# likojack/bnv_fusion

Hardware: AMD Instinct MI355X
Metric: depth frames/sec fused+decoded, 640x480 @ 256^3 grid (higher is better)
Workload: dtype f32 operands split into f16 hi+lo, 3 products on v_mfma_f32_16x16x32_f16, f32 accumulate

## Files before the change

### bnv_fusion_amd/csrc/encode.hip

```cpp
#include <stddef.h>

#include <atomic>
#include <utility>
#include <vector>

#include "frontend.hpp"
#include "tcnn_mlp.hpp"

namespace bnv {

int g_num_cus = 0;
int g_last_hip_error = 0;
std::atomic<int> g_reserve_cus{0};
std::atomic<int> g_finalize_blocks{0};
std::atomic<int> g_tcnn_shared_table{1};
std::atomic<int> g_tcnn_block_encoder{1};
std::atomic<int> g_mlp_mode{1};

bool g_prof_on = false;
static std::vector<std::pair<hipEvent_t, hipEvent_t>> g_prof_events[PROF_KINDS];
static size_t g_prof_used[PROF_KINDS] = {0, 0, 0, 0};

void prof_mark(int kind, bool begin, hipStream_t stream) {
  auto& ring = g_prof_events[kind];
// ... 827 lines not shown
    const bool have = tile_pair(T, t, j, &i, &k);
    float in0 = 0.f, in1 = 0.f, in2 = 0.f;
    int slot = -1;
    bool valid = false;
    if (have) {
      const float* p = pts + (size_t)i * 6;
      const float x = p[0], y = p[1], z = p[2];
      valid = in_bounds(x, y, z, g);
      if (valid) {
        const float xn = voxel_coord(x, g.bound_min[0], g.voxel_size);
        const float yn = voxel_coord(y, g.bound_min[1], g.voxel_size);
        const float zn = voxel_coord(z, g.bound_min[2], g.voxel_size);
        const int gx = (k & 1) ? (int)ceilf(xn) : (int)floorf(xn);
        const int gy = (k & 2) ? (int)ceilf(yn) : (int)floorf(yn);
        const int gz = (k & 4) ? (int)ceilf(zn) : (int)floorf(zn);
        if (voxel_owner(gx, gy, gz, g) == g.shard_rank) {
          const uint32_t id = (uint32_t)(gx * nyz + gy * g.n_xyz[2] + gz);
          const uint32_t word = bitmap[id >> 5];
          slot = (int)(word_prefix[id >> 5] + __popc(word & ((1u << (id & 31)) - 1u)));
        }
        const float rx = relative_coord(xn, gx, g.voxel_size);
        const float ry = relative_coord(yn, gy, g.voxel_size);
        const float rz = relative_coord(zn, gz, g.voxel_size);
        in0 = h ? ry : rx;
        in1 = h ? p[3] : rz;
        in2 = h ? p[5] : p[4];
      }
    }
    if (__ballot(slot >= 0) == 0ULL) continue;

    f32x16 ha[4], hb[4];
#pragma unroll
    for (int mb = 0; mb < 4; ++mb) ha[mb] = bias_init(lds + PN_B1, mb, h);
    {
      const float bin[3] = {in0, in1, in2};
#pragma unroll
      for (int s = 0; s < 3; ++s) {
#pragma unroll
        for (int mb = 0; mb < 4; ++mb)
          ha[mb] = __builtin_amdgcn_mfma_f32_32x32x2f32(lds[PN_W1 + (s * 4 + mb) * 64 + lane], bin[s],
                                                        ha[mb], 0, 0, 0);
      }
    }
#pragma unroll
    for (int mb = 0; mb < 4; ++mb) ha[mb] = relu16(ha[mb]);
    layer128(lds + PN_W2, lds + PN_B2, ha, hb, lane, h);
#pragma unroll
    for (int mb = 0; mb < 4; ++mb) hb[mb] = relu16(hb[mb]);
    layer128(lds + PN_W3, lds + PN_B3, hb, ha, lane, h);
#pragma unroll
    for (int mb = 0; mb < 4; ++mb) ha[mb] = relu16(ha[mb]);
    f32x16 o;
#pragma unroll
    for (int r = 0; r < 16; ++r) o[r] = 0.f;
    {
      const f32x4 b4 = *(const f32x4*)&lds[PN_B4 + 4 * h];
#pragma unroll
      for (int r = 0; r < 4; ++r) o[r] = b4[r];
    }
#pragma unroll
    for (int nb = 0; nb < 4; ++nb) {
#pragma unroll
      for (int rq = 0; rq < 4; ++rq) {
        f32x4 a = {0.f, 0.f, 0.f, 0.f};
        if (j < 8) a = *(const f32x4*)&lds[PN_W4 + ((((nb * 4 + rq) * 2 + h) * 8) + j) * 4];
#pragma unroll
        for (int i = 0; i < 4; ++i)
          o = __builtin_amdgcn_mfma_f32_32x32x2f32(a[i], ha[nb][4 * rq + i], o, 0, 0, 0);
      }
    }
    scatter_tile(o, slot, j, h, counts, acc);
  }
}


typedef __attribute__((address_space(3))) const half8 lds_half8_t;
typedef __attribute__((address_space(3))) const f32x4 lds_f32x4_t;
constexpr int kLdsWin = 61440;

#ifdef BNV_PHASE_PROF
__device__ unsigned long long g_enc_phase[8 * 16];
#define BNV_EPH(i)                                                                          \
  do {                                                                                      \
    if ((threadIdx.x & 63) == 0) {                                                          \
      unsigned long long* _p = (unsigned long long*)((char*)lds + PX_LDS_BYTES) + (threadIdx.x >> 6) * 16; \
      const unsigned long long _t = clock64();                                              \
      _p[i] += _t - _p[15];                                                                 \
      _p[15] = _t;                                                                          \
    }                                                                                       \
  } while (0)
constexpr int kEncProfLds = 8 * 16 * 8;
#else
#define BNV_EPH(i)
constexpr int kEncProfLds = 0;
#endif

struct EncLdsX {
  uint32_t w[3];
  uint32_t b;
};
__device__ __forceinline__ half8 ldsx_wfrag(const EncLdsX& L, int byte_off) {
  const int b = byte_off / kLdsWin;
  return *(lds_half8_t*)((b == 0 ? L.w[0] : (b == 1 ? L.w[1] : L.w[2])) + (uint32_t)(byte_off - b * kLdsWin));
}
__device__ __forceinline__ f32x4 ldsx_bias(const EncLdsX& L, int layer, int rb) {
  return *(lds_f32x4_t*)(L.b + (uint32_t)((layer * 128 + rb * 16) * 4));
}

template <int NPROD>
__device__ __forceinline__ void layer128_x(const EncLdsX& L, int w_off, int layer, const half8 (&inh)[4][2],
                                           const half8 (&inl)[4][2], f32x4 (&out)[8][2]) {
#pragma unroll
  for (int rb = 0; rb < 8; ++rb) out[rb][0] = out[rb][1] = ldsx_bias(L, layer, rb);
  half8 ah[2], al[2];
#define BNV_LOAD_WX(q)                                                        \
  {                                                                           \
    const int wb = (w_off + (q) * 2 * 64 * 8) * 2;                            \
    ah[(q) & 1] = ldsx_wfrag(L, wb);                                          \
    if (NPROD == 3) al[(q) & 1] = ldsx_wfrag(L, wb + 1024);                   \
  }
  BNV_LOAD_WX(0);
#pragma unroll
  for (int q = 0; q < 32; ++q) {
    if (q + 1 < 32) BNV_LOAD_WX(q + 1);
    __builtin_amdgcn_sched_barrier(0);
    const int s = q >> 3, rb = q & 7;
    if constexpr (NPROD == 3) {
      out[rb][0] = __builtin_amdgcn_mfma_f32_16x16x32_f16(al[q & 1], inh[s][0], out[rb][0], 0, 0, 0);
      out[rb][1] = __builtin_amdgcn_mfma_f32_16x16x32_f16(al[q & 1], inh[s][1], out[rb][1], 0, 0, 0);
      out[rb][0] = __builtin_amdgcn_mfma_f32_16x16x32_f16(ah[q & 1], inl[s][0], out[rb][0], 0, 0, 0);
      out[rb][1] = __builtin_amdgcn_mfma_f32_16x16x32_f16(ah[q & 1], inl[s][1], out[rb][1], 0, 0, 0);
    }
    out[rb][0] = __builtin_amdgcn_mfma_f32_16x16x32_f16(ah[q & 1], inh[s][0], out[rb][0], 0, 0, 0);
    out[rb][1] = __builtin_amdgcn_mfma_f32_16x16x32_f16(ah[q & 1], inh[s][1], out[rb][1], 0, 0, 0);
    __builtin_amdgcn_sched_barrier(0);
  }
#undef BNV_LOAD_WX
}

template <int NPROD>
__device__ __forceinline__ void split_x(const f32x4 (&acc)[8][2], half8 (&oh)[4][2], half8 (&ol)[4][2]) {
#pragma unroll
  for (int s = 0; s < 4; ++s)
#pragma unroll
    for (int cb = 0; cb < 2; ++cb) {
      float x[8];
#pragma unroll
      for (int e = 0; e < 8; ++e) x[e] = relu_bits(acc[2 * s + (e >> 2)][cb][e & 3]);
      if (NPROD == 3) {
        split8_f16(x, oh[s][cb], ol[s][cb]);
      } else {
#pragma unroll
        for (int e = 0; e < 8; ++e) oh[s][cb][e] = (_Float16)x[e];
      }
    }
}

__device__ __forceinline__ void scatter_tile_x(const f32x4& o, int slot, int n, int g, int32_t* __restrict__ counts,
                                               long long* __restrict__ acc) {
  uint32_t lo[4], hi[4];
#pragma unroll
  for (int q = 0; q < 4; ++q) {
    const float r = __builtin_rintf(o[q] * kFixedScale);
    const float hf = __builtin_floorf(r * (1.0f / kFixedScale));
    hi[q] = (uint32_t)(int)hf;
    lo[q] = (uint32_t)__builtin_fmaf(hf, -kFixedScale, r);
  }
#define BNV_SCAN_STEP(ctrl)                                                      \
  "v_add_co_u32_dpp %0, vcc, %0, %0 " ctrl "\n"                                  \
  "v_addc_co_u32_dpp %1, vcc, %1, %1, vcc " ctrl "\n"                            \
  "v_add_co_u32_dpp %2, vcc, %2, %2 " ctrl "\n"                                  \
  "v_addc_co_u32_dpp %3, vcc, %3, %3, vcc " ctrl "\n"                            \
  "v_add_co_u32_dpp %4, vcc, %4, %4 " ctrl "\n"                                  \
  "v_addc_co_u32_dpp %5, vcc, %5, %5, vcc " ctrl "\n"                            \
  "v_add_co_u32_dpp %6, vcc, %6, %6 " ctrl "\n"                                  \
  "v_addc_co_u32_dpp %7, vcc, %7, %7, vcc " ctrl "\n"
  asm volatile("s_nop 1\n"
               BNV_SCAN_STEP("row_shr:1 row_mask:0xf bank_mask:0xf bound_ctrl:1")
               BNV_SCAN_STEP("row_shr:2 row_mask:0xf bank_mask:0xf bound_ctrl:1")
               BNV_SCAN_STEP("row_shr:4 row_mask:0xf bank_mask:0xf bound_ctrl:1")
               BNV_SCAN_STEP("row_shr:8 row_mask:0xf bank_mask:0xf bound_ctrl:1")
               : "+v"(lo[0]), "+v"(hi[0]), "+v"(lo[1]), "+v"(hi[1]), "+v"(lo[2]), "+v"(hi[2]), "+v"(lo[3]), "+v"(hi[3])
               :
               : "vcc");
#undef BNV_SCAN_STEP
  {
    const int tsrc = ((g & 1) * 16 + 15) * 4;
#pragma unroll
    for (int q = 0; q < 4; ++q) {
      const uint32_t tl = (uint32_t)__builtin_amdgcn_ds_bpermute(tsrc, (int)lo[q]);
      const uint32_t th = (uint32_t)__builtin_amdgcn_ds_bpermute(tsrc, (int)hi[q]);
      if (g >= 2) {
        const unsigned long long v = (((unsigned long long)hi[q] << 32) | lo[q]) + (((unsigned long long)th << 32) | tl);
        lo[q] = (uint32_t)v;
        hi[q] = (uint32_t)(v >> 32);
      }
    }
  }
  const int p = (g >> 1) * 16 + n;
  const int slot15 = __builtin_amdgcn_readlane(slot, 15);
  const int prev_row = __builtin_amdgcn_update_dpp(0, slot, 0x111 , 0xf, 0xf, false);
  const int prev = n == 0 ? slot15 : prev_row;
  const unsigned long long heads64 = __ballot(p == 0 || prev != slot);
  const uint32_t heads = ((uint32_t)heads64 & 0xffffu) | (((uint32_t)(heads64 >> 32) & 0xffffu) << 16);
  const int s = 31 - __clz((int)(heads & (0xffffffffu >> (31 - p))));
  const bool is_end = p == 31 || ((heads >> (p + 1)) & 1u);
  const int sp = s > 0 ? s - 1 : 0;
  const int src = (((sp >> 4) * 2 + (g & 1)) * 16 + (sp & 15)) * 4;
  uint32_t plo[4], phi[4];
#pragma unroll
  for (int q = 0; q < 4; ++q) {
    plo[q] = (uint32_t)__builtin_amdgcn_ds_bpermute(src, (int)lo[q]);
    phi[q] = (uint32_t)__builtin_amdgcn_ds_bpermute(src, (int)hi[q]);
  }
#ifdef BNV_PROBE_NO_SCATTER
  if ((blockIdx.x & 63) != 0) return;
#endif
  if (slot >= 0 && is_end) {
    unsigned long long* dst = (unsigned long long*)acc + ((uint32_t)slot * 8u + 4u * (uint32_t)(g & 1));
#pragma unroll
    for (int q = 0; q < 4; ++q) {
      unsigned long long v = ((unsigned long long)hi[q] << 32) | lo[q];
      if (s > 0) v -= ((unsigned long long)phi[q] << 32) | plo[q];
      atomicAdd(dst + q, v);
    }
    if ((g & 1) == 0) atomicAdd(&counts[slot], p - s + 1);
  }
}

template <int NPROD>
__global__ __launch_bounds__(512, 2) __attribute__((amdgpu_num_vgpr(120))) void k_pointnet_scatter_x(
    const float* __restrict__ pts, int n_points, bnv_grid_t g, const float* __restrict__ wpack,
    const uint32_t* __restrict__ bitmap, const uint32_t* __restrict__ word_prefix,
    int32_t* __restrict__ counts, long long* __restrict__ acc, int32_t* __restrict__ error,
    const int32_t* __restrict__ pair_list, const int32_t* __restrict__ n_pairs) {
  extern __shared__ __attribute__((aligned(16))) float lds[];
  const float n_cert = wpack[PN_CERT];
  float* lb = lds + PX_TOTAL / 2;
  for (int i = threadIdx.x; i < 128 * 3 + 8; i += 512) lb[i] = wpack[PN_B1 + i];
  stage_to_lds<512>(wpack + PX_OFF, lds, PX_TOTAL * 2);
  int* tile_ctr = (int*)((char*)lds + PX_TOTAL * 2 + (128 * 3 + 8) * 4);
  if (threadIdx.x == 0) *tile_ctr = 0;
  __syncthreads();

  const int lane = threadIdx.x & 63;
  const int n = lane & 15, gk = lane >> 4;
  const int pair = (gk >> 1) * 16 + n;
  const PairTiles T = pair_tiles(n_points, pair_list, n_pairs);
  const int n_tiles = T.n_tiles;
  const int nyz = g.n_xyz[1] * g.n_xyz[2];
  EncLdsX L;
  {
    const uint32_t lds0 = (uint32_t)(uintptr_t)(__attribute__((address_space(3))) float*)lds;
    L.w[0] = lds0 + lane * 16;
    L.w[1] = L.w[0] + kLdsWin;
    L.w[2] = L.w[0] + 2 * kLdsWin;
    L.b = lds0 + PX_TOTAL * 2 + gk * 16;
    asm volatile("" : "+v"(L.w[0]), "+v"(L.w[1]), "+v"(L.w[2]), "+v"(L.b));
  }

  const int tstep = gridDim.x * 8;
  auto grab = [&]() -> int {
    int c = 0;
    if (lane == 0) c = atomicAdd(tile_ctr, 1);
    c = __builtin_amdgcn_readfirstlane(c);
    return blockIdx.x * 8 + (c & 7) + (c >> 3) * tstep;
  };
  float raw[6];
  int raw_k = 0;
  bool raw_ok = false;
  float nin[6];
  uint32_t n_id = 0, n_word = 0, n_pref = 0;
  bool n_own = false;
  auto stage1 = [&](int t) {
    raw_ok = false;
    if (t < n_tiles) {
      int i = 0;
      if (tile_pair(T, t, pair, &i, &raw_k)) {
        const float* p = pts + (size_t)i * 6;
#pragma unroll
        for (int c = 0; c < 6; ++c) raw[c] = p[c];
        raw_ok = true;
      }
    }
  };
  auto stage2 = [&](int t) {
    n_own = false;
#pragma unroll
    for (int c = 0; c < 6; ++c) nin[c] = 0.f;
    if (raw_ok && in_bounds(raw[0], raw[1], raw[2], g)) {
      const int k = raw_k;
      const float xn = voxel_coord(raw[0], g.bound_min[0], g.voxel_size);
      const float yn = voxel_coord(raw[1], g.bound_min[1], g.voxel_size);
      const float zn = voxel_coord(raw[2], g.bound_min[2], g.voxel_size);
      const int gx = (k & 1) ? (int)ceilf(xn) : (int)floorf(xn);
      const int gy = (k & 2) ? (int)ceilf(yn) : (int)floorf(yn);
      const int gz = (k & 4) ? (int)ceilf(zn) : (int)floorf(zn);
      if (voxel_owner(gx, gy, gz, g) == g.shard_rank) {
        n_own = true;
        n_id = (uint32_t)(gx * nyz + gy * g.n_xyz[2] + gz);
        n_word = bitmap[n_id >> 5];
        n_pref = word_prefix[n_id >> 5];
      }
      if ((gk & 1) == 0) {
        nin[0] = relative_coord(xn, gx, g.voxel_size);
        nin[1] = relative_coord(yn, gy, g.voxel_size);
        nin[2] = relative_coord(zn, gz, g.voxel_size);
        nin[3] = raw[3];
        nin[4] = raw[4];
        nin[5] = raw[5];
      }
      if (!(fmaxf(fmaxf(fabsf(raw[3]), fabsf(raw[4])), fabsf(raw[5])) <= n_cert)) *error = 3;
    }
  };
  int t = grab();
  stage1(t);
  stage2(t);
  int t_next = grab(), t_next2 = 0;
  stage1(t_next);
#ifdef BNV_PHASE_PROF
  if ((threadIdx.x & 63) < 16)
    ((unsigned long long*)((char*)lds + PX_LDS_BYTES))[(threadIdx.x >> 6) * 16 + (threadIdx.x & 63)] = 0;
  if ((threadIdx.x & 63) == 0) ((unsigned long long*)((char*)lds + PX_LDS_BYTES))[(threadIdx.x >> 6) * 16 + 15] = clock64();
#endif

  for (; t < n_tiles; t = t_next, t_next = t_next2) {
    float in[6];
#pragma unroll
    for (int c = 0; c < 6; ++c) in[c] = nin[c];
    const int slot = n_own ? (int)(n_pref + __popc(n_word & ((1u << (n_id & 31)) - 1u))) : -1;
    stage2(t_next);
    t_next2 = grab();
    stage1(t_next2);
    __builtin_amdgcn_sched_barrier(0);
    BNV_EPH(0);
    if (__ballot(slot >= 0) == 0ULL) continue;

    f32x4 ha[8][2], hb[8][2];
    {
      half8 bh[2], bl[2];
#pragma unroll
      for (int cb = 0; cb < 2; ++cb) {
        float x[8];
#pragma unroll
        for (int e = 0; e < 8; ++e) x[e] = 0.f;
#pragma unroll
        for (int e = 0; e < 6; ++e) {
          const float other = __shfl(in[e], (lane + 32) & 63, 64);
          x[e] = gk == 0 ? (cb == 0 ? in[e] : other) : 0.f;
        }
        if (NPROD == 3) {
          split8_f16(x, bh[cb], bl[cb]);
        } else {
#pragma unroll
          for (int e = 0; e < 8; ++e) bh[cb][e] = (_Float16)x[e];
        }
      }
#pragma unroll
      for (int rb = 0; rb < 8; ++rb) {
        const half8 ahi = ldsx_wfrag(L, (PX_W1 + rb * 2 * 64 * 8) * 2), alo = ldsx_wfrag(L, (PX_W1 + rb * 2 * 64 * 8) * 2 + 1024);
        const f32x4 b = ldsx_bias(L, 0, rb);
#pragma unroll
        for (int cb = 0; cb < 2; ++cb) {
          f32x4 c = b;
          if constexpr (NPROD == 3) {
            c = __builtin_amdgcn_mfma_f32_16x16x32_f16(alo, bh[cb], c, 0, 0, 0);
            c = __builtin_amdgcn_mfma_f32_16x16x32_f16(ahi, bl[cb], c, 0, 0, 0);
          }
          ha[rb][cb] = __builtin_amdgcn_mfma_f32_16x16x32_f16(ahi, bh[cb], c, 0, 0, 0);
        }
      }
    }
    BNV_EPH(1);
    half8 sh[4][2], sl[4][2];
    split_x<NPROD>(ha, sh, sl);
    BNV_EPH(2);
    layer128_x<NPROD>(L, PX_W2, 1, sh, sl, hb);
    BNV_EPH(3);
    split_x<NPROD>(hb, sh, sl);
    BNV_EPH(4);
    layer128_x<NPROD>(L, PX_W3, 2, sh, sl, ha);
    BNV_EPH(5);
    split_x<NPROD>(ha, sh, sl);
    BNV_EPH(6);
    f32x4 o[2];
    o[0] = o[1] = *(lds_f32x4_t*)(L.b + 384 * 4);
    {
      half8 w4h[4], w4l[4];
      __builtin_amdgcn_sched_barrier(0);
#pragma unroll
      for (int s = 0; s < 4; ++s) {
        w4h[s] = ldsx_wfrag(L, (PX_W4 + s * 2 * 64 * 8) * 2);
        if (NPROD == 3) w4l[s] = ldsx_wfrag(L, (PX_W4 + s * 2 * 64 * 8) * 2 + 1024);
      }
#pragma unroll
      for (int s = 0; s < 4; ++s) {
#pragma unroll
        for (int cb = 0; cb < 2; ++cb) {
          if constexpr (NPROD == 3) {
            o[cb] = __builtin_amdgcn_mfma_f32_16x16x32_f16(w4l[s], sh[s][cb], o[cb], 0, 0, 0);
            o[cb] = __builtin_amdgcn_mfma_f32_16x16x32_f16(w4h[s], sl[s][cb], o[cb], 0, 0, 0);
          }
          o[cb] = __builtin_amdgcn_mfma_f32_16x16x32_f16(w4h[s], sh[s][cb], o[cb], 0, 0, 0);
        }
      }
    }
    f32x4 mine;
#pragma unroll
    for (int i = 0; i < 4; ++i) {
      const float other = __shfl(o[1][i], (lane + 32) & 63, 64);
      mine[i] = gk < 2 ? o[0][i] : other;
    }
    BNV_EPH(7);
    scatter_tile_x(mine, slot, n, gk, counts, acc);
    BNV_EPH(8);
  }
#ifdef BNV_PHASE_PROF
  if ((threadIdx.x & 63) < 15)
    atomicAdd(&g_enc_phase[(threadIdx.x >> 6) * 16 + (threadIdx.x & 63)],
              ((unsigned long long*)((char*)lds + PX_LDS_BYTES))[(threadIdx.x >> 6) * 16 + (threadIdx.x & 63)]);
#endif
}

typedef TcnnPack<1> PointPack;

__global__ __launch_bounds__(256) void k_pointnet_scatter_t(
    const float* __restrict__ pts, int n_points, bnv_grid_t g, const float* __restrict__ wpack,
    const uint32_t* __restrict__ bitmap, const uint32_t* __restrict__ word_prefix,
    int32_t* __restrict__ counts, long long* __restrict__ acc, const int32_t* __restrict__ pair_list,
    const int32_t* __restrict__ n_pairs) {
  __shared__ __attribute__((aligned(16))) _Float16 wh[PointPack::TOTAL];
  stage_to_lds<256>(wpack, wh, PointPack::TOTAL * 2);
  __syncthreads();
  const int lane = threadIdx.x & 63;
  const int wave = __builtin_amdgcn_readfirstlane(threadIdx.x >> 6);
  const int j = lane & 31, h = lane >> 5;
  const PairTiles T = pair_tiles(n_points, pair_list, n_pairs);
  const int n_tiles = T.n_tiles;
  const int nyz = g.n_xyz[1] * g.n_xyz[2];
  for (int t = blockIdx.x * 4 + wave; t < n_tiles; t += gridDim.x * 4) {
    int i = 0, k = 0;
    const bool have = tile_pair(T, t, j, &i, &k);
    half8 b;
#pragma unroll
    for (int e = 0; e < 8; ++e) b[e] = (_Float16)1.0f;
    int slot = -1;
    bool valid = false;
    if (have) {
      const float* p = pts + (size_t)i * 6;
      const float x = p[0], y = p[1], z = p[2];
      if (in_bounds(x, y, z, g)) {
        valid = true;
        const float xn = voxel_coord(x, g.bound_min[0], g.voxel_size);
        const float yn = voxel_coord(y, g.bound_min[1], g.voxel_size);
        const float zn = voxel_coord(z, g.bound_min[2], g.voxel_size);
        const int gx = (k & 1) ? (int)ceilf(xn) : (int)floorf(xn);
        const int gy = (k & 2) ? (int)ceilf(yn) : (int)floorf(yn);
        const int gz = (k & 4) ? (int)ceilf(zn) : (int)floorf(zn);
        if (voxel_owner(gx, gy, gz, g) == g.shard_rank) {
          const uint32_t id = (uint32_t)(gx * nyz + gy * g.n_xyz[2] + gz);
          const uint32_t word = bitmap[id >> 5];
          slot = (int)(word_prefix[id >> 5] + __popc(word & ((1u << (id & 31)) - 1u)));
        }
        if (h == 0) {
          b[0] = (_Float16)relative_coord(xn, gx, g.voxel_size);
          b[1] = (_Float16)relative_coord(yn, gy, g.voxel_size);
          b[2] = (_Float16)relative_coord(zn, gz, g.voxel_size);
          b[3] = (_Float16)p[3];
        } else {
          b[0] = (_Float16)p[4];
          b[1] = (_Float16)p[5];
        }
      }
    }
    if (__ballot(slot >= 0) == 0ULL) continue;
    (void)valid;
    const half8 x[1] = {b};
    f32x16 o = tcnn_forward<1>(wh, lane, x);
#pragma unroll
    for (int q = 0; q < 4; ++q) o[q] = (float)(_Float16)o[q];
    scatter_tile(o, slot, j, h, counts, acc);
  }
}

constexpr int kAccProbes = 6;
constexpr int kTbWaves = 8;
constexpr int kAccCap = 64 * kTbWaves;
struct WgAcc {
  int key[kAccCap];
  int cnt[kAccCap];
  unsigned long long sum[kAccCap][8];
};

template <bool SHARED>
__global__ __launch_bounds__(64 * kTbWaves) void k_pointnet_scatter_tb(
    const float* __restrict__ pts, int n_points, int frame_w, bnv_grid_t g, const float* __restrict__ wpack,
    const uint32_t* __restrict__ bitmap, const uint32_t* __restrict__ word_prefix, int32_t* __restrict__ counts,
    long long* __restrict__ acc) {
  __shared__ __attribute__((aligned(16))) _Float16 wh[PointPack::TOTAL];
  __shared__ WgAcc T;
  const int lane = threadIdx.x & 63;
  const int wave = __builtin_amdgcn_readfirstlane(threadIdx.x >> 6);
  constexpr int kSpan = SHARED ? kAccCap : 64;
  constexpr int kHashShift = SHARED ? 32 - 9 : 32 - 6;
  static_assert(kAccCap == 512, "hash width");
  const int t_base = SHARED ? 0 : wave * 64;
  T.key[threadIdx.x] = -1;
  T.cnt[threadIdx.x] = 0;
#pragma unroll
  for (int f = 0; f < 8; ++f) T.sum[threadIdx.x][f] = 0ull;
  stage_to_lds<64 * kTbWaves>(wpack, wh, PointPack::TOTAL * 2);
  __syncthreads();
  const int j = lane & 31, h = lane >> 5;
  const int nyz = g.n_xyz[1] * g.n_xyz[2];
  const bool sharded = g.shard_world > 1;
  const bool image = frame_w > 0 && n_points % frame_w == 0;
  const int frame_h = image ? n_points / frame_w : 1;
  const int bw = image ? (frame_w + 7) >> 3 : 0, bh = image ? (frame_h + 3) >> 2 : 0;
  const int n_blocks = image ? bw * bh : (n_points + 31) >> 5;
  const int uw = (bw + 1) >> 1;
  const int n_units = (SHARED && image) ? uw * ((bh + 3) >> 2) : (n_blocks + kTbWaves - 1) / kTbWaves;
  auto flush_entry = [&](int e) {
    const int key = T.key[e];
    if (key >= 0) {
      unsigned long long* dst = (unsigned long long*)acc + (uint32_t)key * 8u;
#pragma unroll
      for (int f = 0; f < 8; ++f) {
        atomicAdd(dst + f, T.sum[e][f]);
        T.sum[e][f] = 0ull;
      }
      atomicAdd(&counts[key], T.cnt[e]);
      T.key[e] = -1;
      T.cnt[e] = 0;
    }
  };
  for (int u = blockIdx.x; u < n_units; u += gridDim.x) {
    int i = -1;
    if (SHARED && image) {
      const int uy = u / uw, ux = u - uy * uw;
      const int by = uy * 4 + (wave >> 1), bx = ux * 2 + (wave & 1);
      const int x = bx * 8 + (j & 7), y = by * 4 + (j >> 3);
      if (bx < bw && x < frame_w && y < frame_h) i = y * frame_w + x;
    } else if (image) {
      const int b = u * kTbWaves + wave;
      const int by = b / bw, bx = b - by * bw;
      const int x = bx * 8 + (j & 7), y = by * 4 + (j >> 3);
      if (b < n_blocks && x < frame_w && y < frame_h) i = y * frame_w + x;
    } else if ((u * kTbWaves + wave) * 32 + j < n_points) {
      i = (u * kTbWaves + wave) * 32 + j;
    }
    bool valid = false;
    float px = 0.f, py = 0.f, pz = 0.f, n0 = 0.f, n1 = 0.f, n2 = 0.f;
    if (i >= 0) {
      const float* p = pts + (size_t)i * 6;
      px = p[0], py = p[1], pz = p[2], n0 = p[3], n1 = p[4], n2 = p[5];
      valid = in_bounds(px, py, pz, g);
    }
    if (__ballot(valid) != 0ULL) {
    int lo3[3] = {0, 0, 0}, hi3[3] = {0, 0, 0};
    _Float16 rl[3], rh[3];
    {
      const float c3[3] = {px, py, pz};
#pragma unroll
      for (int a = 0; a < 3; ++a) {
        const float xn = valid ? voxel_coord(c3[a], g.bound_min[a], g.voxel_size) : 0.f;
        lo3[a] = (int)floorf(xn);
        hi3[a] = (int)ceilf(xn);
        rl[a] = (_Float16)relative_coord(xn, lo3[a], g.voxel_size);
        rh[a] = (_Float16)relative_coord(xn, hi3[a], g.voxel_size);
      }
    }
    uint32_t bw8[8], pf8[8], id8[8];
    bool own8[8];
#pragma unroll
    for (int k = 0; k < 8; ++k) {
      const int gx = (k & 1) ? hi3[0] : lo3[0], gy = (k & 2) ? hi3[1] : lo3[1], gz = (k & 4) ? hi3[2] : lo3[2];
      id8[k] = (uint32_t)(gx * nyz + gy * g.n_xyz[2] + gz);
      bw8[k] = 0u;
      pf8[k] = 0u;
      own8[k] = valid && (!sharded || voxel_owner(gx, gy, gz, g) == g.shard_rank);
      if (own8[k]) {
        bw8[k] = bitmap[id8[k] >> 5];
        pf8[k] = word_prefix[id8[k] >> 5];
      }
    }
    const _Float16 hn0 = (_Float16)n0, hn1 = (_Float16)n1, hn2 = (_Float16)n2;
#pragma unroll
    for (int k = 0; k < 8; ++k) {
      const int slot = own8[k] ? (int)(pf8[k] + __popc(bw8[k] & ((1u << (id8[k] & 31)) - 1u))) : -1;
      if (sharded && __ballot(slot >= 0) == 0ULL) continue;
      half8 bop;
#pragma unroll
      for (int e = 0; e < 8; ++e) bop[e] = (_Float16)1.0f;
      if (valid) {
        if (h == 0) {
          bop[0] = (k & 1) ? rh[0] : rl[0];
          bop[1] = (k & 2) ? rh[1] : rl[1];
          bop[2] = (k & 4) ? rh[2] : rl[2];
          bop[3] = hn0;
        } else {
          bop[0] = hn1;
          bop[1] = hn2;
        }
      }
      const half8 x[1] = {bop};
      f32x16 o = tcnn_forward<1>(wh, lane, x);
#pragma unroll
      for (int q = 0; q < 4; ++q) o[q] = (float)(_Float16)o[q];
      unsigned long long v[4];
      bool is_end;
      int len;
      tile_run_sums(o, slot, j, h, v, is_end, len);
      if (slot >= 0 && is_end) {
        int p = (int)(((uint32_t)slot * 0x9E3779B1u) >> kHashShift), found = -1;
        for (int probe = 0; probe < kAccProbes; ++probe) {
          const int old = atomicCAS(&T.key[t_base + p], -1, slot);
          if (old == -1 || old == slot) {
            found = t_base + p;
            break;
          }
          p = (p + 1) & (kSpan - 1);
        }
        if (found >= 0) {
#pragma unroll
          for (int q = 0; q < 4; ++q) atomicAdd(&T.sum[found][4 * h + q], v[q]);
          if (h == 0) atomicAdd(&T.cnt[found], len);
        } else {
          unsigned long long* dst = (unsigned long long*)acc + ((uint32_t)slot * 8u + 4u * (uint32_t)h);
#pragma unroll
          for (int q = 0; q < 4; ++q) atomicAdd(dst + q, v[q]);
          if (h == 0) atomicAdd(&counts[slot], len);
        }
      }
    }
    }
    if constexpr (SHARED) {
      __syncthreads();
      flush_entry(threadIdx.x);
      __syncthreads();
    } else {
      flush_entry(t_base + lane);
    }
  }
}

__global__ __launch_bounds__(kFinTile) void k_finalize(
    bnv_grid_t g, int emit_all, uint32_t* __restrict__ bitmap, int32_t* __restrict__ ids,
    int32_t* __restrict__ counts, long long* __restrict__ acc, uint64_t* __restrict__ tile_state, uint32_t epoch,
    EncCtl* __restrict__ ctl, const int32_t* __restrict__ valid_blocks, int n_mark_blocks,
    float* __restrict__ out_feats, int64_t* __restrict__ out_pcounts,
    int64_t* __restrict__ out_flat, int64_t* __restrict__ out_grid, int64_t out_capacity,
    bnv_encode_counters_t* __restrict__ counters) {
  __shared__ uint32_t wave_tot[kFinTile / 64];
  __shared__ uint32_t s_excl;
  const int64_t n = ctl->n_unique;
  if (n == 0) {
    if (blockIdx.x == 0 && threadIdx.x == 0) {
      counters->n_valid_points = 0;
      counters->n_unique = 0;
      counters->n_out = 0;
      counters->n_avg_pts = 0.f;
      counters->error = ctl->error;
      counters->reserved[0] = counters->reserved[1] = counters->reserved[2] = 0;
      ctl->error = 0;
      ctl->n_pairs = 0;
      ctl->n_orphans = 0;
      ctl->n_deferred = 0;
    }
    if (blockIdx.x == 0 && threadIdx.x < 64) ctl->shard_boundary[threadIdx.x] = 0;
    return;
  }
  for (int64_t tile = blockIdx.x; tile * kFinTile < n; tile += gridDim.x) {
  if (tile != (int64_t)blockIdx.x) __syncthreads();
  const int64_t sl = tile * kFinTile + threadIdx.x;
  ValidFlags flags{counts, ids, g, emit_all};
  const uint32_t fl = sl < n ? flags(sl) : 0u;
  int id = 0, c = 0;
  long long a8[8] = {0, 0, 0, 0, 0, 0, 0, 0};
  bool dirty = false;
  if (sl < n) {
    id = ids[sl];
    c = counts[sl];
    dirty = g.shard_world <= 1 || c != 0;
    if (dirty) {
      typedef long long i64x2 __attribute__((ext_vector_type(2)));
#pragma unroll
      for (int q = 0; q < 4; ++q) {
        const i64x2 v = *(const i64x2*)&acc[sl * 8 + 2 * q];
        a8[2 * q] = v[0];
        a8[2 * q + 1] = v[1];
      }
    }
  }
  uint32_t total;
  uint32_t run = block_exclusive_scan<kFinTile>(fl, wave_tot, &total);
  const bool last_tile = (tile + 1) * kFinTile >= n;
  if (threadIdx.x < 64) {
    const uint32_t excl = lookback_exclusive(tile_state, (int)tile, total, epoch);
    if (threadIdx.x == 0) s_excl = excl;
    if (last_tile) {
      int nv = 0;
      for (int b = threadIdx.x; b < n_mark_blocks; b += 64) nv += valid_blocks[b];
#pragma unroll
      for (int d = 32; d >= 1; d >>= 1) nv += __shfl_xor(nv, d, 64);
      if (threadIdx.x == 0) {
        const int32_t n_out = (int32_t)(excl + total);
        counters->n_valid_points = nv;
        counters->n_unique = (int32_t)n;
        counters->n_out = n_out;
        counters->n_avg_pts = __fdiv_rn((float)(8 * nv), (float)n);
        counters->error = ctl->error ? ctl->error : ((int64_t)n_out > out_capacity ? 2 : 0);
        counters->reserved[0] = ctl->n_pairs;
        counters->reserved[1] = counters->reserved[2] = 0;
        ctl->n_unique = 0;
// ... 389 lines not shown
```

### bnv_fusion_amd/weights.py

```python
import os

import numpy as np

_HERE = os.path.dirname(os.path.abspath(__file__))
DEFAULT_FP32 = os.path.join(_HERE, "weights", "pointnet_fp32.npz")
DEFAULT_TCNN = os.path.join(_HERE, "weights", "pointnet_tcnn.npz")

BN_EPS = 1e-5


def load_npz(path=DEFAULT_FP32):
    with np.load(path) as z:
        return {k: z[k] for k in z.files}


def _np(v):
    return v.detach().cpu().numpy() if hasattr(v, "detach") else np.asarray(v)


def fold_pointnet(sd):
    out = []
    for i in (1, 2, 3, 4):
        p = "pointnet_backbone."
        W = _np(sd[f"{p}conv{i}.weight"]).astype(np.float64)[:, :, 0]
        b = _np(sd[f"{p}conv{i}.bias"]).astype(np.float64)
        s = _np(sd[f"{p}bn{i}.weight"]).astype(np.float64) / np.sqrt(
            _np(sd[f"{p}bn{i}.running_var"]).astype(np.float64) + BN_EPS)
        Wf = W * s[:, None]
        bf = (b - _np(sd[f"{p}bn{i}.running_mean"]).astype(np.float64)) * s + _np(sd[f"{p}bn{i}.bias"]).astype(
            np.float64)
        out.append((Wf.astype(np.float32), bf.astype(np.float32)))
    return out


F16_MAX = 65504.0


def certified_input_bound(layers, fixed, n_free, limit=0.98 * F16_MAX):
    W0 = np.abs(np.asarray(layers[0][0], dtype=np.float64))
    fixed = np.asarray(fixed, dtype=np.float64)
    k = len(fixed)
    assert W0.shape[1] == k + n_free
    a = W0[:, :k] @ fixed + np.abs(np.asarray(layers[0][1], dtype=np.float64))
    c = W0[:, k:].sum(1)
    best = np.inf
    for i, (W, b) in enumerate(layers):
        if i:
            Wa = np.abs(np.asarray(W, dtype=np.float64))
            a, c = Wa @ a + np.abs(np.asarray(b, dtype=np.float64)), Wa @ c
        if (a >= limit).any():
            return 0.0
        with np.errstate(divide="ignore"):
            best = min(best, float(np.min(np.where(c > 0, (limit - a) / c, np.inf))))
    return best


def pointnet_normal_bound(sd):
    return certified_input_bound(fold_pointnet(sd)[:3], [1.0, 1.0, 1.0], 3)


def sdf_feature_bound(sd):
    layers = [(_np(sd[f"nerf.geo_layer{i}.weight"]), _np(sd[f"nerf.geo_layer{i}.bias"])) for i in range(3)]
    return certified_input_bound(layers, [1.5] * 3 + [1.0] * 6, 8)


def pack_pointnet(sd):
    (W1, b1), (W2, b2), (W3, b3), (W4, b4) = fold_pointnet(sd)
    lane = np.arange(64)
    n, h = lane & 31, lane >> 5
    w1p = np.zeros((3, 4, 64), np.float32)
    for s in range(3):
        for mb in range(4):
            w1p[s, mb] = W1[mb * 32 + n, 2 * s + h]

    def pack128(W):
        o = np.zeros((4, 4, 4, 64, 4), np.float32)
        for mb in range(4):
            for nb in range(4):
                for rq in range(4):
                    for i in range(4):
                        o[mb, nb, rq, :, i] = W[mb * 32 + n, nb * 32 + 8 * rq + i + 4 * h]
        return o

    w4p = np.zeros((4, 4, 2, 8, 4), np.float32)
    for nb in range(4):
        for rq in range(4):
            for hh in range(2):
                for i in range(4):
                    w4p[nb, rq, hh, :, i] = W4[:, nb * 32 + 8 * rq + i + 4 * hh]
    fp32_part = np.concatenate([w1p.ravel(), pack128(W2).ravel(), pack128(W3).ravel(), w4p.ravel(),
                                b1, b2, b3, b4]).astype(np.float32)
    trailer = np.zeros(4, np.float32)
    trailer[0] = min(pointnet_normal_bound(sd), 3.0e38)
    return np.concatenate([fp32_part, _pack_pointnet_split16(W1, W2, W3, W4), trailer])


def split_f16(x):
    x = np.asarray(x, dtype=np.float32)
    hi = x.astype(np.float16)
    lo = (x - hi.astype(np.float32)).astype(np.float16)
    return hi, lo


def _slot_feature(jj, h):
    return 8 * (jj >> 2) + 4 * h + (jj & 3)


def _pack_pointnet_split16(W1, W2, W3, W4):
    lane = np.arange(64)
    m, g = lane & 15, lane >> 4
    jj = np.arange(8)
    W1p = np.zeros((128, 32), np.float32)
    W1p[:, :6] = W1
    w1 = np.zeros((8, 2, 64, 8), np.float16)
    for rb in range(8):
        w1[rb, 0], w1[rb, 1] = split_f16(W1p[(16 * rb + m)[:, None], 8 * g[:, None] + jj[None, :]])

    def kidx(s):
        return 32 * s + 16 * (jj[None, :] >> 2) + 4 * g[:, None] + (jj[None, :] & 3)

    def pack128(W):
        o = np.zeros((4, 8, 2, 64, 8), np.float16)
        for s in range(4):
            for rb in range(8):
                o[s, rb, 0], o[s, rb, 1] = split_f16(W[(16 * rb + m)[:, None], kidx(s)])
        return o

    W4p = np.zeros((16, 128), np.float32)
    W4p[:8] = W4
    w4 = np.zeros((4, 2, 64, 8), np.float16)
    for s in range(4):
        w4[s, 0], w4[s, 1] = split_f16(W4p[m[:, None], kidx(s)])
    halves = np.concatenate([w1.ravel(), pack128(W2).ravel(), pack128(W3).ravel(), w4.ravel()])
    assert halves.size == 77824
    return halves.view(np.float32)


def _pack_split(W, nks, n_blocks=8):
    lane = np.arange(64)
    n, h = lane & 31, lane >> 5
    Wp = np.zeros((32 * n_blocks, 16 * nks), np.float32)
    Wp[:W.shape[0], :W.shape[1]] = W
    jj = np.arange(8)
    o = np.zeros((n_blocks, nks, 2, 64, 8), np.float16)
    for w in range(n_blocks):
        for ks in range(nks):
            v = Wp[(32 * w + n)[:, None], 16 * ks + _slot_feature(jj[None, :], h[:, None])]
            o[w, ks, 0], o[w, ks, 1] = split_f16(v)
    return o.ravel()


def _pack_split16(W, n_steps, first_layer=False):
    lane = np.arange(64)
    m, g = lane & 15, lane >> 4
    jj = np.arange(8)
    Wp = np.zeros((256, 32 * n_steps), np.float32)
    Wp[:W.shape[0], :W.shape[1]] = W
    o = np.zeros((8, 2 * n_steps, 2, 64, 8), np.float16)
    for w in range(8):
        for s in range(n_steps):
            for rb in range(2):
                if first_layer:
                    k = 8 * g[:, None] + jj[None, :]
                else:
                    k = 32 * s + 16 * (jj[None, :] >> 2) + 4 * g[:, None] + (jj[None, :] & 3)
                v = Wp[(32 * w + 16 * rb + m)[:, None], k]
                o[w, 2 * s + rb, 0], o[w, 2 * s + rb, 1] = split_f16(v)
    return o.ravel()


def pack_sdf_mlp_bwd(sd):
    Ws = [_np(sd[f"nerf.geo_layer{i}.weight"]).astype(np.float32) for i in range(4)]
    halves = np.concatenate([_pack_split(Ws[3].T, 16), _pack_split(Ws[2].T, 16), _pack_split(Ws[1].T, 16),
                             _pack_split(Ws[0].T, 16, n_blocks=1)])
    assert halves.size == 409600
    return halves.view(np.float32).copy()


def pack_sdf_mlp(sd):
    lane = np.arange(64)
    n, h = lane & 31, lane >> 5

    def pack(W, nkb):
        K = W.shape[1]
        o = np.zeros((8, nkb, 64, 4), np.float32)
        for w in range(8):
            for kb in range(nkb):
                for i in range(4):
                    k = 8 * kb + 4 * h + i
                    ok = k < K
                    o[w, kb, ok, i] = W[32 * w + n[ok], k[ok]]
        return o.ravel()

    Ws = [_np(sd[f"nerf.geo_layer{i}.weight"]).astype(np.float32) for i in range(4)]
    bs = [_np(sd[f"nerf.geo_layer{i}.bias"]).astype(np.float32) for i in range(4)]
    assert Ws[0].shape == (256, 17) and all(W.shape == (256, 256) for W in Ws[1:])
    wa = _np(sd["nerf.fc_alpha.weight"]).astype(np.float32).reshape(256)
    ba = np.zeros(4, np.float32)
    ba[0] = _np(sd["nerf.fc_alpha.bias"]).reshape(-1)[0]
    ba[1] = min(sdf_feature_bound(sd), 3.0e38)
    fp32_part = np.concatenate([pack(Ws[0], 3), pack(Ws[1], 32), pack(Ws[2], 32), pack(Ws[3], 32),
                                bs[0], bs[1], bs[2], bs[3], wa, ba]).astype(np.float32)

    halves = np.concatenate([_pack_split(Ws[0], 2), _pack_split(Ws[1], 16), _pack_split(Ws[2], 16),
                             _pack_split(Ws[3], 16)])
    assert halves.size == 409600
    halves_x = np.concatenate([_pack_split16(Ws[0], 1, first_layer=True), _pack_split16(Ws[1], 8),
                               _pack_split16(Ws[2], 8), _pack_split16(Ws[3], 8)])
    assert halves_x.size == 409600
    return np.concatenate([fp32_part, halves.view(np.float32), halves_x.view(np.float32)])


def _split_tcnn(params, n_in_padded, width=64, n_hidden=3):
    params = _np(params).astype(np.float32).reshape(-1)
    dims = [n_in_padded] + [width] * n_hidden + [16]
    mats, off = [], 0
    for i in range(len(dims) - 1):
        mats.append(params[off: off + dims[i + 1] * dims[i]].reshape(dims[i + 1], dims[i]))
        off += dims[i + 1] * dims[i]
    assert off == params.size, (off, params.size)
    return mats


def _pack_tcnn(mats):
    lane = np.arange(64)
    n, h = lane & 31, lane >> 5
    jj = np.arange(8)
    sf = _slot_feature(jj[None, :], h[:, None])
    out = []
    W0 = mats[0]
    nks = W0.shape[1] // 16
    o = np.zeros((2, nks, 64, 8), np.float16)
    for mb in range(2):
        for ks in range(nks):
            o[mb, ks] = W0[(mb * 32 + n)[:, None], 16 * ks + sf]
    out.append(o.ravel())
    for W in mats[1:-1]:
        o = np.zeros((2, 4, 64, 8), np.float16)
        for mb in range(2):
            for g in range(4):
                o[mb, g] = W[(mb * 32 + n)[:, None], (g >> 1) * 32 + 16 * (g & 1) + sf]
        out.append(o.ravel())
    Wl = np.zeros((32, 64), np.float32)
    Wl[:16] = mats[-1]
    o = np.zeros((4, 64, 8), np.float16)
    for g in range(4):
        o[g] = Wl[n[:, None], (g >> 1) * 32 + 16 * (g & 1) + sf]
    out.append(o.ravel())
    return np.concatenate(out).view(np.float32)


def pack_pointnet_tcnn(params):
    return _pack_tcnn(_split_tcnn(params, 16))


def pack_sdf_tcnn(params):
    return _pack_tcnn(_split_tcnn(params, 32))


def pack_sdf_tcnn_bwd(params):
    W0, W1, W2, W3 = _split_tcnn(params, 32)
    h16 = lambda W: W.astype(np.float16).astype(np.float32)
    lane = np.arange(64)
    n, h = lane & 31, lane >> 5
    sf = _slot_feature(np.arange(8)[None, :], h[:, None])
    out = []
    for W in (h16(W2).T, h16(W1).T):
        o = np.zeros((2, 4, 64, 8), np.float16)
        for mb in range(2):
            for g in range(4):
                o[mb, g] = W[(mb * 32 + n)[:, None], (g >> 1) * 32 + 16 * (g & 1) + sf]
        out.append(o.ravel())
    Wt = h16(W0).T
    o = np.zeros((4, 64, 8), np.float16)
    for g in range(4):
        o[g] = Wt[n[:, None], (g >> 1) * 32 + 16 * (g & 1) + sf]
    out.append(o.ravel())
    halves = np.concatenate(out).view(np.float32)
    return np.concatenate([halves, h16(W3)[0].astype(np.float32)])
```

Before: 581.0.

## Pack split-f16 hi/lo products into unused MFMA K-slots for first and last layers

```diff
diff --git a/bnv_fusion_amd/csrc/encode.hip b/bnv_fusion_amd/csrc/encode.hip
--- a/bnv_fusion_amd/csrc/encode.hip
+++ b/bnv_fusion_amd/csrc/encode.hip
@@ -1153,14 +1153,12 @@
         n_word = bitmap[n_id >> 5];
         n_pref = word_prefix[n_id >> 5];
       }
-      if ((gk & 1) == 0) {
-        nin[0] = relative_coord(xn, gx, g.voxel_size);
-        nin[1] = relative_coord(yn, gy, g.voxel_size);
-        nin[2] = relative_coord(zn, gz, g.voxel_size);
-        nin[3] = raw[3];
-        nin[4] = raw[4];
-        nin[5] = raw[5];
-      }
+      nin[0] = relative_coord(xn, gx, g.voxel_size);
+      nin[1] = relative_coord(yn, gy, g.voxel_size);
+      nin[2] = relative_coord(zn, gz, g.voxel_size);
+      nin[3] = raw[3];
+      nin[4] = raw[4];
+      nin[5] = raw[5];
       if (!(fmaxf(fmaxf(fabsf(raw[3]), fabsf(raw[4])), fabsf(raw[5])) <= n_cert)) *error = 3;
     }
   };
@@ -1189,37 +1187,37 @@
 
     f32x4 ha[8][2], hb[8][2];
     {
-      half8 bh[2], bl[2];
+      half8 bop[2];
+      float other[6];
+#pragma unroll
+      for (int e = 0; e < 6; ++e) other[e] = __shfl(in[e], lane ^ 32, 64);
 #pragma unroll
       for (int cb = 0; cb < 2; ++cb) {
         float x[8];
 #pragma unroll
-        for (int e = 0; e < 8; ++e) x[e] = 0.f;
-#pragma unroll
-        for (int e = 0; e < 6; ++e) {
-          const float other = __shfl(in[e], (lane + 32) & 63, 64);
-          x[e] = gk == 0 ? (cb == 0 ? in[e] : other) : 0.f;
+        for (int e = 0; e < 6; ++e) x[e] = (gk >> 1) == cb ? in[e] : other[e];
+        x[6] = x[7] = 0.f;
+        half8 xh, xl;
+        if (NPROD == 3) {
+          split8_f16(x, xh, xl);
+        } else {
+#pragma unroll
+          for (int e = 0; e < 8; ++e) xh[e] = (_Float16)x[e];
         }
-        if (NPROD == 3) {
-          split8_f16(x, bh[cb], bl[cb]);
-        } else {
-#pragma unroll
-          for (int e = 0; e < 8; ++e) bh[cb][e] = (_Float16)x[e];
+#pragma unroll
+        for (int e = 0; e < 8; ++e) {
+          if (NPROD == 3)
+            bop[cb][e] = gk == 3 ? (_Float16)0.f : (gk == 1 ? xl[e] : xh[e]);
+          else
+            bop[cb][e] = gk == 0 ? xh[e] : (_Float16)0.f;
         }
       }
 #pragma unroll
       for (int rb = 0; rb < 8; ++rb) {
-        const half8 ahi = ldsx_wfrag(L, (PX_W1 + rb * 2 * 64 * 8) * 2), alo = ldsx_wfrag(L, (PX_W1 + rb * 2 * 64 * 8) * 2 + 1024);
+        const half8 a = ldsx_wfrag(L, (PX_W1 + rb * 2 * 64 * 8) * 2);
         const f32x4 b = ldsx_bias(L, 0, rb);
 #pragma unroll
-        for (int cb = 0; cb < 2; ++cb) {
-          f32x4 c = b;
-          if constexpr (NPROD == 3) {
-            c = __builtin_amdgcn_mfma_f32_16x16x32_f16(alo, bh[cb], c, 0, 0, 0);
-            c = __builtin_amdgcn_mfma_f32_16x16x32_f16(ahi, bl[cb], c, 0, 0, 0);
-          }
-          ha[rb][cb] = __builtin_amdgcn_mfma_f32_16x16x32_f16(ahi, bh[cb], c, 0, 0, 0);
-        }
+        for (int cb = 0; cb < 2; ++cb) ha[rb][cb] = __builtin_amdgcn_mfma_f32_16x16x32_f16(a, bop[cb], b, 0, 0, 0);
       }
     }
     BNV_EPH(1);
@@ -1235,7 +1233,11 @@
     split_x<NPROD>(ha, sh, sl);
     BNV_EPH(6);
     f32x4 o[2];
-    o[0] = o[1] = *(lds_f32x4_t*)(L.b + 384 * 4);
+    {
+      const f32x4 b4 = *(lds_f32x4_t*)(L.b + 384 * 4);
+#pragma unroll
+      for (int i = 0; i < 4; ++i) o[0][i] = o[1][i] = gk < 2 ? b4[i] : 0.f;
+    }
     {
       half8 w4h[4], w4l[4];
       __builtin_amdgcn_sched_barrier(0);
@@ -1251,16 +1253,18 @@
           if constexpr (NPROD == 3) {
             o[cb] = __builtin_amdgcn_mfma_f32_16x16x32_f16(w4l[s], sh[s][cb], o[cb], 0, 0, 0);
             o[cb] = __builtin_amdgcn_mfma_f32_16x16x32_f16(w4h[s], sl[s][cb], o[cb], 0, 0, 0);
+          } else {
+            o[cb] = __builtin_amdgcn_mfma_f32_16x16x32_f16(w4h[s], sh[s][cb], o[cb], 0, 0, 0);
           }
-          o[cb] = __builtin_amdgcn_mfma_f32_16x16x32_f16(w4h[s], sh[s][cb], o[cb], 0, 0, 0);
         }
       }
     }
     f32x4 mine;
 #pragma unroll
     for (int i = 0; i < 4; ++i) {
-      const float other = __shfl(o[1][i], (lane + 32) & 63, 64);
-      mine[i] = gk < 2 ? o[0][i] : other;
+      const float keep = gk < 2 ? o[0][i] : o[1][i];
+      const float other = __shfl(gk < 2 ? o[1][i] : o[0][i], lane ^ 32, 64);
+      mine[i] = keep + other;
     }
     BNV_EPH(7);
     scatter_tile_x(mine, slot, n, gk, counts, acc);
diff --git a/bnv_fusion_amd/weights.py b/bnv_fusion_amd/weights.py
--- a/bnv_fusion_amd/weights.py
+++ b/bnv_fusion_amd/weights.py
@@ -110,11 +110,11 @@
     lane = np.arange(64)
     m, g = lane & 15, lane >> 4
     jj = np.arange(8)
-    W1p = np.zeros((128, 32), np.float32)
-    W1p[:, :6] = W1
     w1 = np.zeros((8, 2, 64, 8), np.float16)
     for rb in range(8):
-        w1[rb, 0], w1[rb, 1] = split_f16(W1p[(16 * rb + m)[:, None], 8 * g[:, None] + jj[None, :]])
+        hi, lo = split_f16(W1[16 * rb + m])
+        w1[rb, 0, :, :6] = np.where((g < 2)[:, None], hi, np.where((g == 2)[:, None], lo, 0))
+        w1[rb, 1, :, :6] = np.where((g == 0)[:, None], lo, 0)
 
     def kidx(s):
         return 32 * s + 16 * (jj[None, :] >> 2) + 4 * g[:, None] + (jj[None, :] & 3)
@@ -126,11 +126,11 @@
                 o[s, rb, 0], o[s, rb, 1] = split_f16(W[(16 * rb + m)[:, None], kidx(s)])
         return o
 
-    W4p = np.zeros((16, 128), np.float32)
-    W4p[:8] = W4
     w4 = np.zeros((4, 2, 64, 8), np.float16)
     for s in range(4):
-        w4[s, 0], w4[s, 1] = split_f16(W4p[m[:, None], kidx(s)])
+        hi, lo = split_f16(W4[(m & 7)[:, None], kidx(s)])
+        w4[s, 0] = np.where((m < 8)[:, None], hi, 0)
+        w4[s, 1] = np.where((m < 8)[:, None], lo, hi)
     halves = np.concatenate([w1.ravel(), pack128(W2).ravel(), pack128(W3).ravel(), w4.ravel()])
     assert halves.size == 77824
     return halves.view(np.float32)
```

After: 572.8. 0.986x the previous value.
